# chanchanchan97/ICAFusion

Measured on AMD Instinct MI355X. Metric: RGB/IR image-pairs/sec (two-stream forward + NMS), higher is better.
Workload: dtype bf16

## Files before the change

icafusion_amd/csrc/pool.hip:

```cpp
#include "icaf_common.h"
#include <cstdlib>
#include <algorithm>
#include <cstdint>

namespace icaf {

template <int DT>
__global__ __launch_bounds__(256) void preprocess_kernel(const float* __restrict__ img, typename Elem<DT>::type* __restrict__ out,
                                                         int B, int C, int H, int W, int Cpad, int mode) {
    using E = Elem<DT>;
    const int Ho = mode ? H / 2 : H, Wo = mode ? W / 2 : W;
    const long long npix = (long long)B * Ho * Wo;
    const int nv = Cpad / E::VEC;
    for (long long pix = (long long)blockIdx.x * blockDim.x + threadIdx.x; pix < npix; pix += (long long)gridDim.x * blockDim.x) {
        const int wo = (int)(pix % Wo);
        const long long t = pix / Wo;
        const int ho = (int)(t % Ho), b = (int)(t / Ho);
        for (int v = 0; v < nv; ++v) {
            float f[E::VEC];
#pragma unroll
            for (int j = 0; j < E::VEC; ++j) {
                const int ch = v * E::VEC + j;
                float val = 0.0f;
                if (mode == 0) {
                    if (ch < C) val = img[(((long long)b * C + ch) * H + ho) * W + wo];
                } else if (ch < 4 * C) {
                    const int sub = ch / C, c = ch - sub * C, dy = sub >> 1, dx = sub & 1;
                    val = img[(((long long)b * C + c) * H + 2 * ho + dy) * W + 2 * wo + dx];
                }
                f[j] = val;
            }
            *(u32x4*)(out + pix * Cpad + v * E::VEC) = pack16<DT>(f);
        }
    }
}

template <int DT>
__global__ __launch_bounds__(256) void preprocess_u8_kernel(const unsigned char* __restrict__ img, typename Elem<DT>::type* __restrict__ out,
                                                            int B, int Ctot, int c0, int C, int nstreams, int H, int W, int Cpad, int mode) {
    using E = Elem<DT>;
    const int Ho = mode ? H / 2 : H, Wo = mode ? W / 2 : W;
    const long long npix = (long long)nstreams * B * Ho * Wo;
    const int nv = Cpad / E::VEC;
    for (long long pix = (long long)blockIdx.x * blockDim.x + threadIdx.x; pix < npix; pix += (long long)gridDim.x * blockDim.x) {
        const int wo = (int)(pix % Wo);
        long long t = pix / Wo;
        const int ho = (int)(t % Ho);
        t /= Ho;
        const int b = (int)(t % B), st = (int)(t / B);
        const unsigned char* src = img + ((long long)b * Ctot + c0 + st * C) * H * W;
        for (int v = 0; v < nv; ++v) {
            float f[E::VEC];
#pragma unroll
            for (int j = 0; j < E::VEC; ++j) {
                const int ch = v * E::VEC + j;
                float val = 0.0f;
                if (mode == 0) {
                    if (ch < C) val = (float)src[((long long)ch * H + ho) * W + wo] / 255.0f;
                } else if (ch < 4 * C) {
                    const int sub = ch / C, c = ch - sub * C, dy = sub >> 1, dx = sub & 1;
                    val = (float)src[((long long)c * H + 2 * ho + dy) * W + 2 * wo + dx] / 255.0f;
                }
                f[j] = val;
            }
            *(u32x4*)(out + pix * Cpad + v * E::VEC) = pack16<DT>(f);
        }
    }
}


template <int DT>
__global__ __launch_bounds__(256) void sppf_kernel(const typename Elem<DT>::type* __restrict__ x, int ldx,
                                                   typename Elem<DT>::type* __restrict__ y1, typename Elem<DT>::type* __restrict__ y2,
                                                   typename Elem<DT>::type* __restrict__ y3, int ldy, int B, int H, int W, int C, int k) {
    using E = Elem<DT>;
    const int nv = C / E::VEC;
    const long long total = (long long)B * H * W * nv;
    const int r1 = k / 2, r2 = 2 * r1, r3 = 3 * r1;
    for (long long idx = (long long)blockIdx.x * blockDim.x + threadIdx.x; idx < total; idx += (long long)gridDim.x * blockDim.x) {
        const int v = (int)(idx % nv);
        const long long pix = idx / nv;
        const int w = (int)(pix % W);
        const long long t = pix / W;
        const int h = (int)(t % H), b = (int)(t / H);
        float m1[E::VEC], m2[E::VEC], m3[E::VEC];
#pragma unroll
        for (int j = 0; j < E::VEC; ++j) m1[j] = m2[j] = m3[j] = -INFINITY;
        for (int dy = -r3; dy <= r3; ++dy) {
            const int hh = h + dy;
            if ((unsigned)hh >= (unsigned)H) continue;
            const int ady = dy < 0 ? -dy : dy;
            for (int dx = -r3; dx <= r3; ++dx) {
                const int ww = w + dx;
                if ((unsigned)ww >= (unsigned)W) continue;
                const int adx = dx < 0 ? -dx : dx;
                const int rad = ady > adx ? ady : adx;
                float f[E::VEC];
                unpack16<DT>(*(const u32x4*)(x + (((long long)b * H + hh) * W + ww) * ldx + v * E::VEC), f);
#pragma unroll
                for (int j = 0; j < E::VEC; ++j) {
                    m3[j] = fmaxf(m3[j], f[j]);
                    if (rad <= r2) m2[j] = fmaxf(m2[j], f[j]);
                    if (rad <= r1) m1[j] = fmaxf(m1[j], f[j]);
                }
            }
        }
        const long long o = pix * ldy + v * E::VEC;
        *(u32x4*)(y1 + o) = pack16<DT>(m1);
        *(u32x4*)(y2 + o) = pack16<DT>(m2);
        *(u32x4*)(y3 + o) = pack16<DT>(m3);
    }
}


__device__ __forceinline__ unsigned int key16x2(unsigned int b) {
    const unsigned int sign = b & 0x80008000u;
    return b ^ ((sign >> 15) * 0x7fffu | 0x80008000u);
}
__device__ __forceinline__ u32x4 key_vec(u32x4 v) { return u32x4{key16x2(v[0]), key16x2(v[1]), key16x2(v[2]), key16x2(v[3])}; }
__device__ __forceinline__ unsigned int unkey16x2(unsigned int k) {
    const unsigned int pos = k & 0x80008000u;
    return k ^ (((pos ^ 0x80008000u) >> 15) * 0x7fffu | 0x80008000u);
}
__device__ __forceinline__ u32x4 unkey_vec(u32x4 v) { return u32x4{unkey16x2(v[0]), unkey16x2(v[1]), unkey16x2(v[2]), unkey16x2(v[3])}; }
__device__ __forceinline__ unsigned int max_u16x2(unsigned int a, unsigned int b) {
    using u16x2 = __attribute__((ext_vector_type(2))) unsigned short;
    const u16x2 x = __builtin_bit_cast(u16x2, a), y = __builtin_bit_cast(u16x2, b);
    const u16x2 m = __builtin_elementwise_max(x, y);
    return __builtin_bit_cast(unsigned int, m);
}

template <int DT> struct PlaneMax {
    static __device__ __forceinline__ u32x4 in(u32x4 v) { return key_vec(v); }
    static __device__ __forceinline__ u32x4 out(u32x4 v) { return unkey_vec(v); }
    static __device__ __forceinline__ u32x4 mx(u32x4 a, u32x4 b) {
        return u32x4{max_u16x2(a[0], b[0]), max_u16x2(a[1], b[1]), max_u16x2(a[2], b[2]), max_u16x2(a[3], b[3])};
    }
};
template <> struct PlaneMax<ICAF_F32> {
    static __device__ __forceinline__ u32x4 in(u32x4 v) { return v; }
    static __device__ __forceinline__ u32x4 out(u32x4 v) { return v; }
    static __device__ __forceinline__ u32x4 mx(u32x4 a, u32x4 b) {
        u32x4 r;
#pragma unroll
        for (int j = 0; j < 4; ++j) r[j] = __float_as_uint(fmaxf(__uint_as_float(a[j]), __uint_as_float(b[j])));
        return r;
    }
};

template <int DT>
__global__ __launch_bounds__(256) void sppf_lds_kernel(const typename Elem<DT>::type* __restrict__ x, int ldx,
                                                       typename Elem<DT>::type* __restrict__ y1, typename Elem<DT>::type* __restrict__ y2,
                                                       typename Elem<DT>::type* __restrict__ y3, int ldy, int H, int W, int C, int k,
                                                       int vpb) {
    using E = Elem<DT>;
    using PM = PlaneMax<DT>;
    extern __shared__ __attribute__((aligned(16))) unsigned char smem[];
    u32x4* cur = (u32x4*)smem;
    u32x4* tmp = cur + (size_t)H * W * vpb;
    const int nvb = (C / E::VEC) / vpb;
    const int b = blockIdx.x / nvb, vg = blockIdx.x - b * nvb;
    const int n = H * W * vpb, r = k / 2;
    const long long pix0 = (long long)b * H * W;
    constexpr int MAXIT = 8;
    short iv[MAXIT], ix[MAXIT], iy[MAXIT];
#pragma unroll
    for (int t = 0; t < MAXIT; ++t) {
        const int i = threadIdx.x + t * 256;
        const int ii = i < n ? i : 0;
        const int v = ii % vpb, pp = ii / vpb;
        iv[t] = (short)v; ix[t] = (short)(pp % W); iy[t] = (short)(pp / W);
    }
#pragma unroll
    for (int t = 0; t < MAXIT; ++t) {
        const int i = threadIdx.x + t * 256;
        if (i < n) cur[i] = PM::in(*(const u32x4*)(x + (pix0 + iy[t] * W + ix[t]) * ldx + (vg * vpb + iv[t]) * E::VEC));
    }
    __syncthreads();
    typename E::type* outs[3] = {y1, y2, y3};
#pragma unroll
    for (int stage = 0; stage < 3; ++stage) {
#pragma unroll
        for (int t = 0; t < MAXIT; ++t) {
            const int i = threadIdx.x + t * 256;
            if (i >= n) continue;
            const int xx = ix[t];
            u32x4 m = cur[i];
            for (int d = -r; d <= r; ++d) {
                if (d == 0 || (unsigned)(xx + d) >= (unsigned)W) continue;
                m = PM::mx(m, cur[i + d * vpb]);
            }
            tmp[i] = m;
        }
        __syncthreads();
#pragma unroll
        for (int t = 0; t < MAXIT; ++t) {
            const int i = threadIdx.x + t * 256;
            if (i >= n) continue;
            const int yy = iy[t];
            u32x4 m = tmp[i];
            for (int d = -r; d <= r; ++d) {
                if (d == 0 || (unsigned)(yy + d) >= (unsigned)H) continue;
                m = PM::mx(m, tmp[i + d * W * vpb]);
            }
            cur[i] = m;
            *(u32x4*)(outs[stage] + (pix0 + yy * W + ix[t]) * ldy + (vg * vpb + iv[t]) * E::VEC) = PM::out(m);
        }
        __syncthreads();
    }
}

struct UpsampleDiv { FastDiv nv, wo, ho, scale; };

template <bool I32>
__global__ __launch_bounds__(256) void upsample_kernel(const u32x4* __restrict__ x, int ldxv, u32x4* __restrict__ y, int ldyv,
                                                       int B, int H, int W, int nv, int scale, UpsampleDiv dv) {
    const int Ho = H * scale, Wo = W * scale;
    const long long total = (long long)B * Ho * Wo * nv;
    for (long long idx = (long long)blockIdx.x * blockDim.x + threadIdx.x; idx < total; idx += (long long)gridDim.x * blockDim.x) {
        if constexpr (I32) {
            unsigned int pix, v, t, wo, b, ho;
            fd_divmod((unsigned int)idx, dv.nv, pix, v);
            fd_divmod(pix, dv.wo, t, wo);
            fd_divmod(t, dv.ho, b, ho);
            const unsigned int hi = fd_div(ho, dv.scale), wi = fd_div(wo, dv.scale);
            y[(long long)pix * ldyv + v] = x[(((long long)b * H + hi) * W + wi) * ldxv + v];
        } else {
            const int v = (int)(idx % nv);
            const long long pix = idx / nv;
            const int wo = (int)(pix % Wo);
            const long long t = pix / Wo;
            const int ho = (int)(t % Ho), b = (int)(t / Ho);
            y[pix * ldyv + v] = x[(((long long)b * H + ho / scale) * W + wo / scale) * ldxv + v];
        }
    }
}

__global__ __launch_bounds__(256) void copy_kernel(const u32x4* __restrict__ x, int ldxv, u32x4* __restrict__ y, int ldyv,
                                                   long long rows, int nv) {
    const long long total = rows * nv;
    for (long long idx = (long long)blockIdx.x * blockDim.x + threadIdx.x; idx < total; idx += (long long)gridDim.x * blockDim.x) {
        const int v = (int)(idx % nv);
        const long long r = idx / nv;
        y[r * ldyv + v] = x[r * ldxv + v];
    }
}

template <int DT>
__global__ __launch_bounds__(256) void axpby_kernel(const typename Elem<DT>::type* __restrict__ x0, int ld0,
                                                    const typename Elem<DT>::type* __restrict__ x1, int ld1,
                                                    typename Elem<DT>::type* __restrict__ y, int ldy, long long rows, int nv, float a, float b) {
    using E = Elem<DT>;
    const long long total = rows * nv;
    for (long long idx = (long long)blockIdx.x * blockDim.x + threadIdx.x; idx < total; idx += (long long)gridDim.x * blockDim.x) {
        const int v = (int)(idx % nv);
        const long long r = idx / nv;
        float f0[E::VEC], f1[E::VEC], o[E::VEC];
        unpack16<DT>(*(const u32x4*)(x0 + r * ld0 + v * E::VEC), f0);
        unpack16<DT>(*(const u32x4*)(x1 + r * ld1 + v * E::VEC), f1);
#pragma unroll
        for (int j = 0; j < E::VEC; ++j) o[j] = f0[j] * a + f1[j] * b;
        *(u32x4*)(y + r * ldy + v * E::VEC) = pack16<DT>(o);
    }
}

static inline unsigned grid_for(long long total) {
    long long b = (total + 255) / 256;
    if (b > 256 * 16) b = 256 * 16;
    if (b < 1) b = 1;
    return (unsigned)b;
}

static inline int vec_of(int dtype) { return dtype == ICAF_F32 ? 4 : 8; }

}

using namespace icaf;

extern "C" int icaf_preprocess_nchw(const float* img, void* out, int dtype, int B, int C, int H, int W, int Cpad, int mode,
                                    icaf_stream_t s) {
    if (!img || !out) return fail(ICAF_ERR_ARG, "icaf_preprocess_nchw: null pointer");
    if (dtype < 0 || dtype > 2) return fail(ICAF_ERR_ARG, "icaf_preprocess_nchw: bad dtype");
    const int vec = vec_of(dtype);
    if (Cpad % vec) return fail(ICAF_ERR_ARG, "icaf_preprocess_nchw: Cpad %d must be a multiple of %d", Cpad, vec);
    if (mode == 1 && ((H | W) & 1)) return fail(ICAF_ERR_ARG, "icaf_preprocess_nchw: space-to-depth needs even H, W");
    if (mode == 1 ? Cpad < 4 * C : Cpad < C) return fail(ICAF_ERR_ARG, "icaf_preprocess_nchw: Cpad too small");
    const long long total = (long long)B * (mode ? H / 2 : H) * (mode ? W / 2 : W);
    dim3 grid(grid_for(total)), block(256);
    if (dtype == ICAF_F32) hipLaunchKernelGGL(preprocess_kernel<ICAF_F32>, grid, block, 0, S(s), img, (float*)out, B, C, H, W, Cpad, mode);
    else if (dtype == ICAF_BF16) hipLaunchKernelGGL(preprocess_kernel<ICAF_BF16>, grid, block, 0, S(s), img, (unsigned short*)out, B, C, H, W, Cpad, mode);
    else hipLaunchKernelGGL(preprocess_kernel<ICAF_F16>, grid, block, 0, S(s), img, (unsigned short*)out, B, C, H, W, Cpad, mode);
    ICAF_LAUNCH_CHECK();
    return ICAF_OK;
}

extern "C" int icaf_preprocess_u8(const unsigned char* img, void* out, int dtype, int B, int Ctot, int c0, int C, int nstreams, int H,
                                  int W, int Cpad, int mode, icaf_stream_t s) {
    if (!img || !out) return fail(ICAF_ERR_ARG, "icaf_preprocess_u8: null pointer");
    if (dtype < 0 || dtype > 2) return fail(ICAF_ERR_ARG, "icaf_preprocess_u8: bad dtype");
    const int vec = vec_of(dtype);
    if (Cpad % vec) return fail(ICAF_ERR_ARG, "icaf_preprocess_u8: Cpad %d must be a multiple of %d", Cpad, vec);
    if (mode == 1 && ((H | W) & 1)) return fail(ICAF_ERR_ARG, "icaf_preprocess_u8: space-to-depth needs even H, W");
    if (mode == 1 ? Cpad < 4 * C : Cpad < C) return fail(ICAF_ERR_ARG, "icaf_preprocess_u8: Cpad too small");
    if (nstreams < 1 || c0 < 0 || c0 + nstreams * C > Ctot) return fail(ICAF_ERR_ARG, "icaf_preprocess_u8: channels [%d, %d) exceed %d", c0, c0 + nstreams * C, Ctot);
    const long long total = (long long)nstreams * B * (mode ? H / 2 : H) * (mode ? W / 2 : W);
    dim3 grid(grid_for(total)), block(256);
    if (dtype == ICAF_F32) hipLaunchKernelGGL(preprocess_u8_kernel<ICAF_F32>, grid, block, 0, S(s), img, (float*)out, B, Ctot, c0, C, nstreams, H, W, Cpad, mode);
    else if (dtype == ICAF_BF16) hipLaunchKernelGGL(preprocess_u8_kernel<ICAF_BF16>, grid, block, 0, S(s), img, (unsigned short*)out, B, Ctot, c0, C, nstreams, H, W, Cpad, mode);
    else hipLaunchKernelGGL(preprocess_u8_kernel<ICAF_F16>, grid, block, 0, S(s), img, (unsigned short*)out, B, Ctot, c0, C, nstreams, H, W, Cpad, mode);
    ICAF_LAUNCH_CHECK();
    return ICAF_OK;
}


static int sppf_select(int dtype, int H, int W, int C) {
    const int nv = C / vec_of(dtype);
    int cap = 8;
    if (g_opt.sppf_vpb > 0) cap = g_opt.sppf_vpb;
    for (int c : {8, 4, 2, 1})
        if (c <= cap && nv % c == 0 && (size_t)H * W * c * 32 <= 60 * 1024) return c;
    return 0;
}

extern "C" int icaf_sppf_config(int dtype, int H, int W, int C, int* vpb) {
    if (!vpb) return fail(ICAF_ERR_ARG, "icaf_sppf_config: null pointer");
    if (dtype < 0 || dtype > 2) return fail(ICAF_ERR_ARG, "icaf_sppf_config: bad dtype");
    if (H < 1 || W < 1 || C < 1 || C % vec_of(dtype)) return fail(ICAF_ERR_ARG, "icaf_sppf_config: bad geometry");
    *vpb = sppf_select(dtype, H, W, C);
    return ICAF_OK;
}

extern "C" int icaf_sppf_pool(const void* x, int ldx, void* y1, void* y2, void* y3, int ldy, int dtype, int B, int H, int W, int C,
                              int k, icaf_stream_t s) {
    if (!x || !y1 || !y2 || !y3) return fail(ICAF_ERR_ARG, "icaf_sppf_pool: null pointer");
    if (dtype < 0 || dtype > 2) return fail(ICAF_ERR_ARG, "icaf_sppf_pool: bad dtype");
    const int vec = vec_of(dtype);
    if (C % vec || ldx % vec || ldy % vec || !(k & 1)) return fail(ICAF_ERR_ARG, "icaf_sppf_pool: C/ld must be multiples of %d and k odd", vec);
    const int nv = C / vec;
    const int vpb = sppf_select(dtype, H, W, C);
    if (vpb) {
        const size_t lds = (size_t)H * W * vpb * 32;
        dim3 grid((unsigned)(B * (nv / vpb))), block(256);
        if (dtype == ICAF_F32) sppf_lds_kernel<ICAF_F32><<<grid, block, lds, S(s)>>>((const float*)x, ldx, (float*)y1, (float*)y2, (float*)y3, ldy, H, W, C, k, vpb);
        else if (dtype == ICAF_BF16) sppf_lds_kernel<ICAF_BF16><<<grid, block, lds, S(s)>>>((const unsigned short*)x, ldx, (unsigned short*)y1, (unsigned short*)y2, (unsigned short*)y3, ldy, H, W, C, k, vpb);
        else sppf_lds_kernel<ICAF_F16><<<grid, block, lds, S(s)>>>((const unsigned short*)x, ldx, (unsigned short*)y1, (unsigned short*)y2, (unsigned short*)y3, ldy, H, W, C, k, vpb);
        ICAF_LAUNCH_CHECK();
        return ICAF_OK;
    }
    const long long total = (long long)B * H * W * (C / vec);
    dim3 grid(grid_for(total)), block(256);
    if (dtype == ICAF_F32) hipLaunchKernelGGL(sppf_kernel<ICAF_F32>, grid, block, 0, S(s), (const float*)x, ldx, (float*)y1, (float*)y2, (float*)y3, ldy, B, H, W, C, k);
    else if (dtype == ICAF_BF16) hipLaunchKernelGGL(sppf_kernel<ICAF_BF16>, grid, block, 0, S(s), (const unsigned short*)x, ldx, (unsigned short*)y1, (unsigned short*)y2, (unsigned short*)y3, ldy, B, H, W, C, k);
    else hipLaunchKernelGGL(sppf_kernel<ICAF_F16>, grid, block, 0, S(s), (const unsigned short*)x, ldx, (unsigned short*)y1, (unsigned short*)y2, (unsigned short*)y3, ldy, B, H, W, C, k);
    ICAF_LAUNCH_CHECK();
    return ICAF_OK;
}

extern "C" int icaf_upsample_nearest(const void* x, int ldx, void* y, int ldy, int dtype, int B, int H, int W, int C, int scale,
                                     icaf_stream_t s) {
    if (!x || !y) return fail(ICAF_ERR_ARG, "icaf_upsample_nearest: null pointer");
    if (dtype < 0 || dtype > 2) return fail(ICAF_ERR_ARG, "icaf_upsample_nearest: bad dtype");
    const int vec = vec_of(dtype);
    if (C % vec || ldx % vec || ldy % vec || scale < 1) return fail(ICAF_ERR_ARG, "icaf_upsample_nearest: bad geometry");
    const long long total = (long long)B * H * scale * W * scale * (C / vec);
    if (total < 1) return fail(ICAF_ERR_ARG, "icaf_upsample_nearest: empty tensor");
    const UpsampleDiv dv{make_fastdiv((unsigned)(C / vec)), make_fastdiv((unsigned)(W * scale)), make_fastdiv((unsigned)(H * scale)),
                         make_fastdiv((unsigned)scale)};
    if (total < (1ll << 31))
        hipLaunchKernelGGL(upsample_kernel<true>, dim3(grid_for(total)), dim3(256), 0, S(s), (const u32x4*)x, ldx / vec, (u32x4*)y,
                           ldy / vec, B, H, W, C / vec, scale, dv);
    else
        hipLaunchKernelGGL(upsample_kernel<false>, dim3(grid_for(total)), dim3(256), 0, S(s), (const u32x4*)x, ldx / vec, (u32x4*)y,
                           ldy / vec, B, H, W, C / vec, scale, dv);
    ICAF_LAUNCH_CHECK();
    return ICAF_OK;
}

extern "C" int icaf_axpby(const void* x0, int ld0, const void* x1, int ld1, void* y, int ldy, int dtype, long long rows, int C, float a,
                          float b, icaf_stream_t s) {
    if (!x0 || !x1 || !y) return fail(ICAF_ERR_ARG, "icaf_axpby: null pointer");
    if (dtype < 0 || dtype > 2) return fail(ICAF_ERR_ARG, "icaf_axpby: bad dtype");
    const int vec = vec_of(dtype);
    if (C % vec || ld0 % vec || ld1 % vec || ldy % vec) return fail(ICAF_ERR_ARG, "icaf_axpby: C/ld must be multiples of %d", vec);
    dim3 grid(grid_for(rows * (C / vec))), block(256);
    if (dtype == ICAF_F32) axpby_kernel<ICAF_F32><<<grid, block, 0, S(s)>>>((const float*)x0, ld0, (const float*)x1, ld1, (float*)y, ldy, rows, C / vec, a, b);
    else if (dtype == ICAF_BF16) axpby_kernel<ICAF_BF16><<<grid, block, 0, S(s)>>>((const unsigned short*)x0, ld0, (const unsigned short*)x1, ld1, (unsigned short*)y, ldy, rows, C / vec, a, b);
    else axpby_kernel<ICAF_F16><<<grid, block, 0, S(s)>>>((const unsigned short*)x0, ld0, (const unsigned short*)x1, ld1, (unsigned short*)y, ldy, rows, C / vec, a, b);
    ICAF_LAUNCH_CHECK();
    return ICAF_OK;
}

extern "C" int icaf_copy_channels(const void* x, int ldx, void* y, int ldy, int dtype, long long rows, int C, icaf_stream_t s) {
    if (!x || !y) return fail(ICAF_ERR_ARG, "icaf_copy_channels: null pointer");
    if (dtype < 0 || dtype > 2) return fail(ICAF_ERR_ARG, "icaf_copy_channels: bad dtype");
    const int vec = vec_of(dtype);
    if (C % vec || ldx % vec || ldy % vec) return fail(ICAF_ERR_ARG, "icaf_copy_channels: C/ld must be multiples of %d", vec);
    hipLaunchKernelGGL(copy_kernel, dim3(grid_for(rows * (C / vec))), dim3(256), 0, S(s), (const u32x4*)x, ldx / vec, (u32x4*)y, ldy / vec,
                       rows, C / vec);
    ICAF_LAUNCH_CHECK();
    return ICAF_OK;
}
```

Measured before the change: 17120.

## Specialize SPPF LDS pooling for k=5 with 512 threads and clamped windows

Adds a k=5 specialized SPPF kernel with 512-thread blocks. It prefetches inputs into registers and computes the separable max with clamped neighbour offsets, which removes the bounds branches. The second and third pooled outputs are built from sparse samples of the first-stage result, so the extra two full passes and barriers disappear. It also swizzles block indices for locality and simplifies the bf16 key transforms with arithmetic sign fill. The price is more code paths, higher register pressure, and a MAXIT limit tied to a 1920-element plane assumption.

```diff
diff --git a/icafusion_amd/csrc/pool.hip b/icafusion_amd/csrc/pool.hip
--- a/icafusion_amd/csrc/pool.hip
+++ b/icafusion_amd/csrc/pool.hip
@@ -113,14 +113,16 @@
 }
 
 
+__device__ __forceinline__ unsigned int sign_fill16x2(unsigned int b) {
+    using i16x2 = __attribute__((ext_vector_type(2))) short;
+    return __builtin_bit_cast(unsigned int, __builtin_bit_cast(i16x2, b) >> 15);
+}
 __device__ __forceinline__ unsigned int key16x2(unsigned int b) {
-    const unsigned int sign = b & 0x80008000u;
-    return b ^ ((sign >> 15) * 0x7fffu | 0x80008000u);
+    return b ^ (sign_fill16x2(b) | 0x80008000u);
 }
 __device__ __forceinline__ u32x4 key_vec(u32x4 v) { return u32x4{key16x2(v[0]), key16x2(v[1]), key16x2(v[2]), key16x2(v[3])}; }
 __device__ __forceinline__ unsigned int unkey16x2(unsigned int k) {
-    const unsigned int pos = k & 0x80008000u;
-    return k ^ (((pos ^ 0x80008000u) >> 15) * 0x7fffu | 0x80008000u);
+    return ~(k ^ (sign_fill16x2(k) & 0x7fff7fffu));
 }
 __device__ __forceinline__ u32x4 unkey_vec(u32x4 v) { return u32x4{unkey16x2(v[0]), unkey16x2(v[1]), unkey16x2(v[2]), unkey16x2(v[3])}; }
 __device__ __forceinline__ unsigned int max_u16x2(unsigned int a, unsigned int b) {
@@ -149,13 +151,11 @@
 };
 
 template <int DT>
-__global__ __launch_bounds__(256) void sppf_lds_kernel(const typename Elem<DT>::type* __restrict__ x, int ldx,
-                                                       typename Elem<DT>::type* __restrict__ y1, typename Elem<DT>::type* __restrict__ y2,
-                                                       typename Elem<DT>::type* __restrict__ y3, int ldy, int H, int W, int C, int k,
-                                                       int vpb) {
+__device__ __forceinline__ void sppf_lds_any_k(unsigned char* smem, const typename Elem<DT>::type* __restrict__ x, int ldx,
+                                               typename Elem<DT>::type* __restrict__ y1, typename Elem<DT>::type* __restrict__ y2,
+                                               typename Elem<DT>::type* __restrict__ y3, int ldy, int H, int W, int C, int k, int vpb) {
     using E = Elem<DT>;
     using PM = PlaneMax<DT>;
-    extern __shared__ __attribute__((aligned(16))) unsigned char smem[];
     u32x4* cur = (u32x4*)smem;
     u32x4* tmp = cur + (size_t)H * W * vpb;
     const int nvb = (C / E::VEC) / vpb;
@@ -208,6 +208,119 @@
         }
         __syncthreads();
     }
+}
+
+constexpr int SPPF_NT = 512;
+
+__device__ __forceinline__ unsigned int sppf_block(unsigned int bid, unsigned int nblk, int lsh) {
+    const int sh = 3 + lsh;
+    if (lsh == 0 || bid >= (nblk >> sh << sh)) return bid;
+    const unsigned int q = bid >> sh, r = bid & ((1u << sh) - 1);
+    return (((q << 3) + (r & 7)) << lsh) + (r >> 3);
+}
+
+template <int DT, int K>
+__device__ __forceinline__ void sppf_lds_fixed_k(unsigned char* smem, const typename Elem<DT>::type* __restrict__ x, int ldx,
+                                                 typename Elem<DT>::type* __restrict__ y1, typename Elem<DT>::type* __restrict__ y2,
+                                                 typename Elem<DT>::type* __restrict__ y3, int ldy, int H, int W, int C, int vpb,
+                                                 int lsh, FastDiv fw) {
+    using E = Elem<DT>;
+    using PM = PlaneMax<DT>;
+    constexpr int R = K / 2;
+    constexpr int MAXIT = (1920 + SPPF_NT - 1) / SPPF_NT;
+    u32x4* cur = (u32x4*)smem;
+    u32x4* tmp = cur + (size_t)H * W * vpb;
+    const int nvb = (C / E::VEC) / vpb;
+    const int blk = (int)sppf_block(blockIdx.x, gridDim.x, lsh);
+    const int b = blk / nvb, vg = blk - b * nvb;
+    const int n = H * W * vpb, lv = __builtin_ctz(vpb), sx = vpb, sy = W * vpb;
+    const long long pix0 = (long long)b * H * W;
+    const char* xg = (const char*)(x + pix0 * ldx + (long long)vg * vpb * E::VEC);
+    const long long og = pix0 * ldy + (long long)vg * vpb * E::VEC;
+    char *y1g = (char*)(y1 + og), *y2g = (char*)(y2 + og), *y3g = (char*)(y3 + og);
+    constexpr unsigned int ES = sizeof(typename E::type);
+    int ix[MAXIT], iy[MAXIT];
+    u32x4 ld[MAXIT];
+#pragma unroll
+    for (int t = 0; t < MAXIT; ++t) {
+        const int i = threadIdx.x + t * SPPF_NT;
+        const unsigned int ii = i < n ? i : 0, p = ii >> lv;
+        const unsigned int yy = fd_div(p, fw);
+        iy[t] = (int)yy; ix[t] = (int)(p - __umul24(yy, W));
+        ld[t] = *(const u32x4*)(xg + (__umul24(p, ldx) + (ii & (vpb - 1)) * E::VEC) * ES);
+    }
+#pragma unroll
+    for (int t = 0; t < MAXIT; ++t) {
+        const int i = threadIdx.x + t * SPPF_NT;
+        if (i < n) cur[i] = PM::in(ld[t]);
+    }
+    __syncthreads();
+#pragma unroll
+    for (int t = 0; t < MAXIT; ++t) {
+        const int i = threadIdx.x + t * SPPF_NT;
+        if (i >= n) continue;
+        const int xl = ix[t], xr = W - 1 - ix[t];
+        u32x4 m = cur[i];
+#pragma unroll
+        for (int d = 1; d <= R; ++d) {
+            m = PM::mx(m, cur[i - __mul24(min(xl, d), sx)]);
+            m = PM::mx(m, cur[i + __mul24(min(xr, d), sx)]);
+        }
+        tmp[i] = m;
+    }
+    __syncthreads();
+#pragma unroll
+    for (int t = 0; t < MAXIT; ++t) {
+        const int i = threadIdx.x + t * SPPF_NT;
+        if (i >= n) continue;
+        const int yu = iy[t], yd = H - 1 - iy[t];
+        u32x4 m = tmp[i];
+#pragma unroll
+        for (int d = 1; d <= R; ++d) {
+            m = PM::mx(m, tmp[i - __mul24(min(yu, d), sy)]);
+            m = PM::mx(m, tmp[i + __mul24(min(yd, d), sy)]);
+        }
+        cur[i] = m;
+        *(u32x4*)(y1g + (__umul24(i >> lv, ldy) + (i & (vpb - 1)) * E::VEC) * ES) = PM::out(m);
+    }
+    __syncthreads();
+#pragma unroll
+    for (int t = 0; t < MAXIT; ++t) {
+        const int i = threadIdx.x + t * SPPF_NT;
+        if (i >= n) continue;
+        const int xl = ix[t], xr = W - 1 - ix[t], yu = iy[t], yd = H - 1 - iy[t];
+        const int xm1 = -__mul24(min(xl, R), sx), xp1 = __mul24(min(xr, R), sx);
+        const int xm2 = -__mul24(min(xl, 2 * R), sx), xp2 = __mul24(min(xr, 2 * R), sx);
+        const int ym1 = -__mul24(min(yu, R), sy), yp1 = __mul24(min(yd, R), sy);
+        const int ym2 = -__mul24(min(yu, 2 * R), sy), yp2 = __mul24(min(yd, 2 * R), sy);
+        const u32x4* c = cur + i;
+        u32x4 m2 = PM::mx(PM::mx(c[ym1 + xm1], c[ym1 + xp1]), PM::mx(c[yp1 + xm1], c[yp1 + xp1]));
+        u32x4 m3 = PM::mx(PM::mx(c[ym2 + xm2], c[ym2]), PM::mx(c[ym2 + xp2], c[xm2]));
+        m3 = PM::mx(PM::mx(m3, c[0]), PM::mx(c[xp2], c[yp2 + xm2]));
+        m3 = PM::mx(m3, PM::mx(c[yp2], c[yp2 + xp2]));
+        const unsigned int o = (__umul24(i >> lv, ldy) + (i & (vpb - 1)) * E::VEC) * ES;
+        *(u32x4*)(y2g + o) = PM::out(m2);
+        *(u32x4*)(y3g + o) = PM::out(m3);
+    }
+}
+
+template <int DT, int K>
+__global__ __launch_bounds__(K ? SPPF_NT : 256) void sppf_lds_kernel(const typename Elem<DT>::type* __restrict__ x, int ldx,
+                                                                     typename Elem<DT>::type* __restrict__ y1,
+                                                                     typename Elem<DT>::type* __restrict__ y2,
+                                                                     typename Elem<DT>::type* __restrict__ y3, int ldy, int H, int W, int C,
+                                                                     int k, int vpb, int lsh, FastDiv fw) {
+    extern __shared__ __attribute__((aligned(16))) unsigned char smem[];
+    if constexpr (K > 0) sppf_lds_fixed_k<DT, K>(smem, x, ldx, y1, y2, y3, ldy, H, W, C, vpb, lsh, fw);
+    else sppf_lds_any_k<DT>(smem, x, ldx, y1, y2, y3, ldy, H, W, C, k, vpb);
+}
+
+struct SppfLdsArgs { const void* x; int ldx; void *y1, *y2, *y3; int ldy, H, W, C, k, vpb, lsh; FastDiv fw; };
+template <int DT, int K>
+static void sppf_lds_launch(dim3 grid, size_t lds, hipStream_t st, const SppfLdsArgs& a) {
+    using T = typename Elem<DT>::type;
+    sppf_lds_kernel<DT, K><<<grid, dim3(K ? SPPF_NT : 256), lds, st>>>((const T*)a.x, a.ldx, (T*)a.y1, (T*)a.y2, (T*)a.y3, a.ldy, a.H, a.W, a.C,
+                                                                       a.k, a.vpb, a.lsh, a.fw);
 }
 
 struct UpsampleDiv { FastDiv nv, wo, ho, scale; };
@@ -340,10 +453,20 @@
     const int vpb = sppf_select(dtype, H, W, C);
     if (vpb) {
         const size_t lds = (size_t)H * W * vpb * 32;
-        dim3 grid((unsigned)(B * (nv / vpb))), block(256);
-        if (dtype == ICAF_F32) sppf_lds_kernel<ICAF_F32><<<grid, block, lds, S(s)>>>((const float*)x, ldx, (float*)y1, (float*)y2, (float*)y3, ldy, H, W, C, k, vpb);
-        else if (dtype == ICAF_BF16) sppf_lds_kernel<ICAF_BF16><<<grid, block, lds, S(s)>>>((const unsigned short*)x, ldx, (unsigned short*)y1, (unsigned short*)y2, (unsigned short*)y3, ldy, H, W, C, k, vpb);
-        else sppf_lds_kernel<ICAF_F16><<<grid, block, lds, S(s)>>>((const unsigned short*)x, ldx, (unsigned short*)y1, (unsigned short*)y2, (unsigned short*)y3, ldy, H, W, C, k, vpb);
+        const int nvb = nv / vpb;
+        int lsh = 0;
+        while ((vpb << (lsh + 1)) <= 8 && nvb % (2 << lsh) == 0) ++lsh;
+        const SppfLdsArgs a{x, ldx, y1, y2, y3, ldy, H, W, C, k, vpb, lsh, make_fastdiv((unsigned)W)};
+        const dim3 grid((unsigned)(B * nvb));
+        if (k == 5 && ldx < (1 << 18) && ldy < (1 << 18)) {
+            if (dtype == ICAF_F32) sppf_lds_launch<ICAF_F32, 5>(grid, lds, S(s), a);
+            else if (dtype == ICAF_BF16) sppf_lds_launch<ICAF_BF16, 5>(grid, lds, S(s), a);
+            else sppf_lds_launch<ICAF_F16, 5>(grid, lds, S(s), a);
+        } else {
+            if (dtype == ICAF_F32) sppf_lds_launch<ICAF_F32, 0>(grid, lds, S(s), a);
+            else if (dtype == ICAF_BF16) sppf_lds_launch<ICAF_BF16, 0>(grid, lds, S(s), a);
+            else sppf_lds_launch<ICAF_F16, 0>(grid, lds, S(s), a);
+        }
         ICAF_LAUNCH_CHECK();
         return ICAF_OK;
     }
```

Result: no change. 17210, median of 6 (+0.5%).
